# lucidrains/imagen-pytorch

Hardware: AMD Instinct MI355X
Metric: images/sec (64->256 cascade, 1000 steps, bs=8) (higher is better)
Workload: dtype f16; 1 GPU; C3: README unet1 (dim 32, 64^2) + unet2 (dim 32, 256^2, lowres_cond) cascade, 1000 DDPM steps/stage, CFG 3.0, dynamic thresholding, batch 8 per GPU; global_batch=8, parallelism=batch-sharded x1, one RCCL all-gather of final images, batch_schedule=5 whole cascades side by side (one stream each), images_in_flight=40, denoiser_evals_per_image=4000

## Files before the change

### imagen-pytorch_amd/csrc/elementwise.hip

```cpp
#include <algorithm>
#include <cstdint>
#include <cstdlib>
#include "common.h"
#include "gca_device.h"

namespace {

__device__ __forceinline__ int lanes_per_row(int groups) {
  int l = 1;
  while (l < groups && l < 64) l <<= 1;
  return l;
}

__device__ __forceinline__ float group_sum(float v, int lpr) {
  for (int off = lpr >> 1; off > 0; off >>= 1) v += __shfl_xor(v, off);
  return v;
}

__global__ __launch_bounds__(256) void rowstat_kernel(const ImagenRowstatParams p, int lpr) {
  const int rows_per_block = 256 / lpr;
  const int sub = threadIdx.x / lpr, li = threadIdx.x % lpr;
  const int r = blockIdx.x * rows_per_block + sub;
  if (r >= p.rows) return;
  const int b = r / p.rows_per_batch, rr = r - b * p.rows_per_batch;
// ... 478 lines not shown
  s_b2[t] = bias2;
  float a = 0.f;
#pragma unroll
  for (int j = 0; j < kGcaFastP; ++j) {
    const int i = sl + j * nsl;
    a += pv[j] * (i < chunks ? s_wgt[i] : 0.f);
  }
  for (int i = sl + kGcaFastP * nsl; i < chunks; i += nsl) a += part[(size_t)i * stride + 2 + c] * s_wgt[i];
  float* red_f = reinterpret_cast<float*>(s_red);
  red_f[t] = a;
  __syncthreads();
  if (t < C) {
    float v = 0.f;
    for (int q = 0; q < nsl; ++q) v += red_f[q * C + t];
    s_ctx[t] = v * inv_S;
  }
  __syncthreads();
  GCA_STAMP(5);
  gca_fast_matvec<W>(w1, w1t, C, hidden, s_ctx, s_red, [&](int o, float v) __attribute__((always_inline)) { s_hid[o] = silu_f(v + s_b1[o]); });
  GCA_STAMP(6);
  gca_fast_matvec<W>(w2, w2t, hidden, C, s_hid, s_red, [&](int o, float v) __attribute__((always_inline)) {
    const float g = sigmoid_f(v + s_b2[o]);
    gate_a[o] = g;
    if (gate_b) gate_b[o] = g;
  });
  GCA_STAMP(7);
}

__global__ __launch_bounds__(kGcaFastThreads) void gca_final_fast_kernel(const ImagenGcaFinalParams p) {
  GCA_STAMP(0);
  gca_final_fast_body<kGcaFastW>(p.part, p.w1t, p.b1, p.w2t, p.b2, blockIdx.x, p.C, p.hidden, p.chunks, p.gate + (size_t)blockIdx.x * p.C, nullptr);
}

template <int PHASE>
__global__ __launch_bounds__(256) void gca_final_split_kernel(const ImagenGcaFinalParams p) {
  __shared__ float s_in[1024], s_wgt[1024], s_red[kGcaScratchFloats];
  const int tid = threadIdx.x, b = blockIdx.y;
  if constexpr (PHASE == 1) {
    gca_merge(p.part + (size_t)b * p.chunks * (p.C + 2), p.chunks, p.C, s_in, s_wgt, s_red);
    const int o = blockIdx.x * 32 + (tid & 31), sl = tid >> 5;
    float a = 0.f;
    if (o < p.hidden) {
      const float* w = p.w1t + o;
#pragma unroll 8
      for (int c = sl; c < p.C; c += 8) a += w[(size_t)c * p.hidden] * s_in[c];
    }
    s_red[tid] = a;
    __syncthreads();
    if (tid < 32 && o < p.hidden) {
      float t = 0.f;
#pragma unroll
      for (int q = 0; q < 8; ++q) t += s_red[q * 32 + tid];
      p.hid[(size_t)b * p.hidden + o] = silu_f(t + p.b1[o]);
    }
  } else {
    for (int i = tid; i < p.hidden; i += 256) s_in[i] = p.hid[(size_t)b * p.hidden + i];
    __syncthreads();
    const int c = blockIdx.x * 64 + (tid & 63), sl = tid >> 6;
    float a = 0.f;
    if (c < p.C) {
      const float* w = p.w2t + c;
#pragma unroll 8
      for (int o = sl; o < p.hidden; o += 4) a += w[(size_t)o * p.C] * s_in[o];
    }
    s_red[tid] = a;
    __syncthreads();
    if (tid < 64 && c < p.C) p.gate[(size_t)b * p.C + c] = sigmoid_f(s_red[tid] + s_red[64 + tid] + s_red[128 + tid] + s_red[192 + tid] + p.b2[c]);
  }
}

__global__ __launch_bounds__(kGcaFastThreads) void gca_tail_kernel(const ImagenGcaTailParams p) {
  GCA_STAMP(0);
  __shared__ float s_gate[1024];
  const int t = threadIdx.x, b = blockIdx.y;
  const int C = p.C, lpr = C >> 3;
  const int rpp = kGcaFastThreads / lpr;
  const int per = (p.HW + (int)gridDim.x - 1) / (int)gridDim.x;
  const int r_begin = blockIdx.x * per, r_end = min(r_begin + per, p.HW);
  const int g = t & (lpr - 1), sub = t / lpr;
  const f16* hb = reinterpret_cast<const f16*>(p.h) + (size_t)b * p.HW * p.ld_h + g * 8;
  const f16* rb = reinterpret_cast<const f16*>(p.res) + (size_t)b * p.HW * p.ld_res + g * 8;
  f16* ob = reinterpret_cast<f16*>(p.out) + (size_t)b * p.HW * p.ld_out + g * 8;
  f16* ab = p.act_out ? reinterpret_cast<f16*>(p.act_out) + (size_t)b * p.HW * p.ld_act + g * 8 : nullptr;
  int r = r_begin + sub;
  f16x8 hv = {}, rv = {};
  if (r < r_end) {
    hv = *reinterpret_cast<const f16x8*>(hb + (size_t)r * p.ld_h);
    rv = *reinterpret_cast<const f16x8*>(rb + (size_t)r * p.ld_res);
  }
  if (p.part) {
    gca_final_fast_body<6>(p.part, p.w1t, p.b1, p.w2t, p.b2, b, C, p.hidden, p.chunks, s_gate, (p.gate && blockIdx.x == 0) ? p.gate + (size_t)b * C : nullptr);
  } else {
    if (t < C) s_gate[t] = p.gate_in ? p.gate_in[(size_t)b * C + t] : 1.0f;
    __syncthreads();
  }
  float4 pa0 = make_float4(0.f, 0.f, 0.f, 0.f), pa1 = pa0;
  if (p.act_pa) {
    pa0 = *reinterpret_cast<const float4*>(p.act_pa + g * 8);
    pa1 = *reinterpret_cast<const float4*>(p.act_pa + g * 8 + 4);
  }
  const float4 g0 = *reinterpret_cast<const float4*>(s_gate + g * 8), g1 = *reinterpret_cast<const float4*>(s_gate + g * 8 + 4);
  const float gt[8] = {g0.x, g0.y, g0.z, g0.w, g1.x, g1.y, g1.z, g1.w};
  const float pa[8] = {pa0.x, pa0.y, pa0.z, pa0.w, pa1.x, pa1.y, pa1.z, pa1.w};
  const float inv_c = 1.0f / (float)C;
  while (r < r_end) {
    const int rn = r + rpp;
    f16x8 hn = {}, rnx = {};
    if (rn < r_end) {
      hn = *reinterpret_cast<const f16x8*>(hb + (size_t)rn * p.ld_h);
      rnx = *reinterpret_cast<const f16x8*>(rb + (size_t)rn * p.ld_res);
    }
    f16x8 o;
    float vr[8], ssq = 0.f, sum = 0.f;
#pragma unroll
    for (int j = 0; j < 8; ++j) {
      o[j] = (f16)((float)hv[j] * gt[j] + (float)rv[j]);
      vr[j] = (float)o[j];
      ssq += vr[j] * vr[j];
      sum += vr[j];
    }
    *reinterpret_cast<f16x8*>(ob + (size_t)r * p.ld_out) = o;
    const size_t row = (size_t)b * p.HW + r;
    if (p.ssq_out || ab) {
      const float tot = group_sum(ssq, lpr);
      if (p.ssq_out && g == 0) p.ssq_out[row] = tot;
      if (ab) {
        const float rs = __builtin_amdgcn_rsqf(fmaxf(tot, 1e-24f));
        f16x8 a;
#pragma unroll
        for (int j = 0; j < 8; ++j) a[j] = (f16)silu_f(vr[j] * rs * pa[j]);
        *reinterpret_cast<f16x8*>(ab + (size_t)r * p.ld_act) = a;
      }
    }
    if (p.mu_out) {
      const float mean = group_sum(sum, lpr) * inv_c;
      float q = 0.f;
#pragma unroll
      for (int j = 0; j < 8; ++j) { const float d = vr[j] - mean; q += d * d; }
      const float var = group_sum(q, lpr) * inv_c;
      if (g == 0) {
        p.mu_out[row] = mean;
        p.rs_out[row] = rsqrtf(var + p.eps);
      }
    }
    hv = hn;
    rv = rnx;
    r = rn;
  }
  GCA_STAMP(8);
}

__global__ __launch_bounds__(256) void time_embed_kernel(const ImagenTimeEmbedParams p) {
  const int i = blockIdx.x * 256 + threadIdx.x;
  if (i >= p.B * p.out_dim) return;
  const int b = i / p.out_dim, o = i - b * p.out_dim;
  int st = p.step_ptr ? *p.step_ptr : 0;
  if (p.steps > 0) st = min(max(st, 0), p.steps - 1);
  const float x = p.step_ptr ? p.coef[(size_t)st * 8 + 6] : p.times[b];
  const int nf = 2 * p.half_dim + 1;
  const float* w = p.w + (size_t)o * nf;
  float a = p.bias[o] + w[0] * x;
  for (int k = 0; k < p.half_dim; ++k) {
    const float f = x * p.freqs[k] * 6.283185307179586f;
    a += w[1 + k] * sinf(f) + w[1 + p.half_dim + k] * cosf(f);
  }
  reinterpret_cast<f16*>(p.hid)[(size_t)b * p.ld_hid + o] = (f16)silu_f(a);
}

__global__ __launch_bounds__(256) void scale_shift_kernel(const ImagenScaleShiftParams p) {
  const int i = blockIdx.x * 256 + threadIdx.x;
  if (i >= p.B * p.total_c) return;
  const int b = i / p.total_c, c = i - b * p.total_c;
  float sc, sh;
  if (p.ss_f32) {
    const float* ss = reinterpret_cast<const float*>(p.ss) + (size_t)b * p.ld_ss;
    sc = ss[p.idx_scale[c]];
    sh = ss[p.idx_shift[c]];
  } else {
    const f16* ss = reinterpret_cast<const f16*>(p.ss) + (size_t)b * p.ld_ss;
    sc = (float)ss[p.idx_scale[c]];
    sh = (float)ss[p.idx_shift[c]];
  }
  p.pa[i] = p.gamma_s[c] * (sc + 1.0f);
  p.ps[i] = sh;
}

constexpr int kLfRows = 16, kLfKc = 128;

__global__ __launch_bounds__(256) void linear_f32_kernel(const ImagenLinearF32Params p) {
  __shared__ float xs[kLfRows][kLfKc];
  const int o = blockIdx.x * 256 + threadIdx.x;
  const int r0 = blockIdx.y * kLfRows;
  const int nr = min(kLfRows, p.rows - r0);
  float acc[kLfRows];
#pragma unroll
  for (int j = 0; j < kLfRows; ++j) acc[j] = 0.f;
  for (int k0 = 0; k0 < p.K; k0 += kLfKc) {
    const int kc = min(kLfKc, p.K - k0);
    __syncthreads();
    for (int i = threadIdx.x; i < kLfRows * kLfKc; i += 256) {
      const int j = i / kLfKc, k = i - j * kLfKc;
      float v = 0.f;
      if (j < nr && k < kc) {
        const size_t at = (size_t)(r0 + j) * p.ld_x + k0 + k;
        v = p.x_f32 ? reinterpret_cast<const float*>(p.x)[at] : (float)reinterpret_cast<const f16*>(p.x)[at];
        if (p.act_in == IMAGEN_ACT_SILU) v = silu_f(v);
      }
      xs[j][k] = v;
    }
    __syncthreads();
    if (o < p.Cout) {
      const float* w = p.wt + (size_t)k0 * p.Cout + o;
      for (int k = 0; k < kc; ++k) {
        const float wv = w[(size_t)k * p.Cout];
#pragma unroll
        for (int j = 0; j < kLfRows; ++j) acc[j] = fmaf(xs[j][k], wv, acc[j]);
      }
    }
  }
  if (o >= p.Cout) return;
  const float b = p.bias ? p.bias[o] : 0.f;
  for (int j = 0; j < nr; ++j) {
    float v = acc[j] + b;
    if (p.res) v += (float)reinterpret_cast<const f16*>(p.res)[(size_t)(r0 + j) * p.ld_res + o];
    p.y[(size_t)(r0 + j) * p.ld_y + o] = v;
  }
}

__global__ __launch_bounds__(256) void pack_image_kernel(const ImagenPackImageParams p) {
  const int i = blockIdx.x * 256 + threadIdx.x;
  const int HW = p.H * p.W;
  if (i >= p.B * p.Brep * HW) return;
  const int bo = i / HW, px = i - bo * HW;
  const int bs = bo % p.B;
  f16* out = reinterpret_cast<f16*>(p.out) + (size_t)i * p.Cpad;
  for (int c = 0; c < p.Cpad; ++c) {
    float v = 0.f;
    if (c < p.Ca) v = p.a[((size_t)bs * p.Ca + c) * HW + px];
    else if (c - p.Ca < p.Cb) v = p.b[((size_t)bs * p.Cb + (c - p.Ca)) * HW + px];
    out[c] = (f16)v;
  }
}

__global__ __launch_bounds__(256) void rows_copy_kernel(const ImagenRowsCopyParams p) {
  const int groups = p.C >> 3;
  const int i = blockIdx.x * 256 + threadIdx.x;
  if (i >= p.B * p.rows * groups) return;
  const int g = i % groups;
  const int r = (i / groups) % p.rows;
  const int b = i / (groups * p.rows);
  const f16* s = reinterpret_cast<const f16*>(p.src) + (size_t)b * p.src_bs + (size_t)r * p.src_rs + g * 8;
  f16* d = reinterpret_cast<f16*>(p.dst) + (size_t)b * p.dst_bs + (size_t)r * p.dst_rs + g * 8;
  *reinterpret_cast<uint4*>(d) = *reinterpret_cast<const uint4*>(s);
}

__global__ __launch_bounds__(256) void select_rows_kernel(const ImagenSelectRowsParams p) {
  const int groups = p.C >> 3;
  const int i = blockIdx.x * 256 + threadIdx.x;
  if (i >= p.R * p.L * groups) return;
  const int g = i % groups;
  const int l = (i / groups) % p.L;
  const int r = i / (groups * p.L);
  const int sb = p.src[r];
  const bool take = p.keep[r] && (p.mask == nullptr || p.mask[(size_t)sb * p.L + l]);
  const f16* s = take ? reinterpret_cast<const f16*>(p.a) + ((size_t)sb * p.L + l) * p.C + g * 8
                      : reinterpret_cast<const f16*>(p.nul) + (size_t)l * p.C + g * 8;
  *reinterpret_cast<uint4*>(reinterpret_cast<f16*>(p.dst) + ((size_t)r * p.L + l) * p.C + g * 8) = *reinterpret_cast<const uint4*>(s);
}

__global__ __launch_bounds__(256) void mean_rows_kernel(const ImagenMeanRowsParams p) {
  const int groups = p.C >> 3;
  const int i = blockIdx.x * 256 + threadIdx.x;
  if (i >= p.B * groups) return;
  const int b = i / groups, g = i - b * groups;
  const f16* x = reinterpret_cast<const f16*>(p.x) + (size_t)b * p.bs_x + g * 8;
  float acc[8] = {0, 0, 0, 0, 0, 0, 0, 0};
  for (int r = 0; r < p.rows; ++r) {
    const f16x8 v = *reinterpret_cast<const f16x8*>(x + (size_t)r * p.ld_x);
#pragma unroll
    for (int j = 0; j < 8; ++j) acc[j] += (float)v[j];
  }
  f16x8 o;
  const float inv = 1.0f / (float)p.rows;
#pragma unroll
  for (int j = 0; j < 8; ++j) o[j] = (f16)(acc[j] * inv);
  *reinterpret_cast<f16x8*>(reinterpret_cast<f16*>(p.out) + (size_t)b * p.ld_out + g * 8) = o;
}

__global__ __launch_bounds__(256) void memset32_kernel(uint32_t* dst, uint32_t value, int count) {
  const int i = blockIdx.x * 256 + threadIdx.x;
  if (i < count) dst[i] = value;
}

inline bool al8(long v) { return v % 8 == 0; }
inline bool al16(const void* q) { return (reinterpret_cast<uintptr_t>(q) & 15) == 0; }
constexpr long kIntMax = 2147483647L;

int host_lpr(int groups) {
  int l = 1;
  while (l < groups && l < 64) l <<= 1;
  return l;
}

__global__ __launch_bounds__(256) void act_prep_kernel(const ImagenActPrepParams p) {
  constexpr int U = 4;
  const int gpp = (p.C1 + p.C2) >> 3;
  const long total = (long)p.rows * gpp;
  const f16* x1 = reinterpret_cast<const f16*>(p.x1);
  const f16* x2 = reinterpret_cast<const f16*>(p.x2);
  f16* y = reinterpret_cast<f16*>(p.y);
  const long stride = (long)gridDim.x * 256;
  for (long i0 = (long)blockIdx.x * 256 + threadIdx.x; i0 < total; i0 += stride * U) {
    f16x8 in[U];
    float rs[U], mu[U], qb[U];
    float4 a0[U], a1[U], s0[U], s1[U];
    f16* dst[U];
#pragma unroll
    for (int u = 0; u < U; ++u) {
      const long i = i0 + u * stride;
      const bool ok = i < total;
      const long ii = ok ? i : 0;
      const int r = (int)(ii / gpp), g = (int)(ii - (long)r * gpp);
      const int b = r / p.rows_per_batch, rr = r - b * p.rows_per_batch;
      const int c0 = g * 8;
      const f16* src = c0 < p.C1 ? x1 + (size_t)b * p.bs1 + (size_t)rr * p.ld1 + c0 : x2 + (size_t)b * p.bs2 + (size_t)rr * p.ld2 + (c0 - p.C1);
      in[u] = *reinterpret_cast<const f16x8*>(src);
      rs[u] = p.rs ? p.rs[r] : (p.ssq_a ? p.ssq_a[r] : 1.0f);
      qb[u] = (!p.rs && p.ssq_b) ? p.ssq_b[r] : 0.0f;
      mu[u] = p.mu ? p.mu[r] : 0.0f;
      const float* pa = p.pa ? p.pa + (size_t)b * p.pstride + c0 : nullptr;
      const float* ps = p.ps ? p.ps + (size_t)b * p.pstride + c0 : nullptr;
      a0[u] = pa ? *reinterpret_cast<const float4*>(pa) : make_float4(1.f, 1.f, 1.f, 1.f);
      a1[u] = pa ? *reinterpret_cast<const float4*>(pa + 4) : make_float4(1.f, 1.f, 1.f, 1.f);
      s0[u] = ps ? *reinterpret_cast<const float4*>(ps) : make_float4(0.f, 0.f, 0.f, 0.f);
      s1[u] = ps ? *reinterpret_cast<const float4*>(ps + 4) : make_float4(0.f, 0.f, 0.f, 0.f);
      dst[u] = ok ? y + (size_t)b * p.bsy + (size_t)rr * p.ldy + c0 : nullptr;
    }
#pragma unroll
    for (int u = 0; u < U; ++u) {
      if (!dst[u]) continue;
      float sc = rs[u];
      if (!p.rs && p.ssq_a) sc = __builtin_amdgcn_rsqf(fmaxf(rs[u] + p.ssq_wb * qb[u], 1e-24f));
      const float a[8] = {a0[u].x, a0[u].y, a0[u].z, a0[u].w, a1[u].x, a1[u].y, a1[u].z, a1[u].w};
      const float sh[8] = {s0[u].x, s0[u].y, s0[u].z, s0[u].w, s1[u].x, s1[u].y, s1[u].z, s1[u].w};
      f16x8 out;
#pragma unroll
      for (int j = 0; j < 8; ++j) {
        float v = ((float)in[u][j] - mu[u]) * sc * a[j] + sh[j];
        if (p.act_in == IMAGEN_ACT_SILU) v = silu_f(v);
        else if (p.act_in == IMAGEN_ACT_GELU) v = gelu_f(v);
        out[j] = (f16)v;
      }
      *reinterpret_cast<f16x8*>(dst[u]) = out;
    }
  }
}

template <int L>
__global__ __launch_bounds__(256) void act_prep_stat_kernel(const ImagenActPrepParams p) {
  const int gpp = (p.C1 + p.C2) >> 3;
  const int g = threadIdx.x % L;
  const int r = blockIdx.x * (256 / L) + threadIdx.x / L;
  const bool live = r < p.rows && g < gpp;
  const int rc = min(r, p.rows - 1), gc = min(g, gpp - 1);
  const int b = rc / p.rows_per_batch, rr = rc - b * p.rows_per_batch;
  const int c0 = gc * 8;
  const f16* x1 = reinterpret_cast<const f16*>(p.x1);
  const f16* x2 = reinterpret_cast<const f16*>(p.x2);
  const f16* src = c0 < p.C1 ? x1 + (size_t)b * p.bs1 + (size_t)rr * p.ld1 + c0 : x2 + (size_t)b * p.bs2 + (size_t)rr * p.ld2 + (c0 - p.C1);
  const f16x8 in = *reinterpret_cast<const f16x8*>(src);
  const float qb = p.ssq_b ? p.ssq_b[rc] : 0.0f;
  const float* pa = p.pa ? p.pa + (size_t)b * p.pstride + c0 : nullptr;
  const float* ps = p.ps ? p.ps + (size_t)b * p.pstride + c0 : nullptr;
  const float4 a0 = pa ? *reinterpret_cast<const float4*>(pa) : make_float4(1.f, 1.f, 1.f, 1.f);
  const float4 a1 = pa ? *reinterpret_cast<const float4*>(pa + 4) : make_float4(1.f, 1.f, 1.f, 1.f);
  const float4 s0 = ps ? *reinterpret_cast<const float4*>(ps) : make_float4(0.f, 0.f, 0.f, 0.f);
  const float4 s1 = ps ? *reinterpret_cast<const float4*>(ps + 4) : make_float4(0.f, 0.f, 0.f, 0.f);
  float own = 0.0f;
  if (live && c0 < p.C1) {
#pragma unroll
    for (int j = 0; j < 8; ++j) own += (float)in[j] * (float)in[j];
  }
#pragma unroll
  for (int o = L / 2; o >= 1; o >>= 1) own += __shfl_xor(own, o);
  if (!live) return;
  const float sc = __builtin_amdgcn_rsqf(fmaxf(own + p.ssq_wb * qb, 1e-24f));
  const float a[8] = {a0.x, a0.y, a0.z, a0.w, a1.x, a1.y, a1.z, a1.w};
  const float sh[8] = {s0.x, s0.y, s0.z, s0.w, s1.x, s1.y, s1.z, s1.w};
  f16x8 out;
#pragma unroll
  for (int j = 0; j < 8; ++j) {
    float v = (float)in[j] * sc * a[j] + sh[j];
    if (p.act_in == IMAGEN_ACT_SILU) v = silu_f(v);
    else if (p.act_in == IMAGEN_ACT_GELU) v = gelu_f(v);
    out[j] = (f16)v;
  }
  *reinterpret_cast<f16x8*>(reinterpret_cast<f16*>(p.y) + (size_t)b * p.bsy + (size_t)rr * p.ldy + c0) = out;
}

__global__ __launch_bounds__(256) void step_slice_kernel(const ImagenStepSliceParams p) {
  int st = *p.step_ptr;
  if (p.steps > 0) st = min(max(st, 0), p.steps - 1);
  const size_t step = (size_t)st;
  const int w0 = p.words0, w1 = w0 + p.words1, w2 = w1 + p.words2, tot = w2 + p.words3;
  for (int i = blockIdx.x * 256 + threadIdx.x; i < tot; i += gridDim.x * 256) {
    const uint4* s;
    uint4* d;
    int j, w;
    if (i < w0) { s = reinterpret_cast<const uint4*>(p.src0); d = reinterpret_cast<uint4*>(p.dst0); j = i; w = p.words0; }
    else if (i < w1) { s = reinterpret_cast<const uint4*>(p.src1); d = reinterpret_cast<uint4*>(p.dst1); j = i - w0; w = p.words1; }
    else if (i < w2) { s = reinterpret_cast<const uint4*>(p.src2); d = reinterpret_cast<uint4*>(p.dst2); j = i - w1; w = p.words2; }
    else { s = reinterpret_cast<const uint4*>(p.src3); d = reinterpret_cast<uint4*>(p.dst3); j = i - w2; w = p.words3; }
    d[j] = s[step * (size_t)w + j];
  }
}

}

#ifdef GCA_TRACE
extern "C" int imagen_debug_gca_trace(void* buf) { return (int)hipMemcpyToSymbol(HIP_SYMBOL(g_gca_trace), &buf, sizeof(buf)); }
#endif

int launch_step_slice(const ImagenStepSliceParams* p, hipStream_t s) {
  IMAGEN_CHECK(p->step_ptr && p->words0 > 0 && p->src0 && p->dst0, "step_slice: null step_ptr / first segment");
  IMAGEN_CHECK((!p->words1 || (p->src1 && p->dst1)) && (!p->words2 || (p->src2 && p->dst2)) && (!p->words3 || (p->src3 && p->dst3)),
               "step_slice: a segment with words but no pointers");
  const long tot = (long)p->words0 + p->words1 + p->words2 + p->words3;
  hipLaunchKernelGGL(step_slice_kernel, dim3((unsigned)std::min<long>((tot + 255) / 256, 2048L)), dim3(256), 0, s, *p);
  return imagen_hip_status("step_slice");
}

int launch_rowstat(const ImagenRowstatParams* p, hipStream_t s) {
  IMAGEN_CHECK(p->C1 % 8 == 0 && p->C2 % 8 == 0 && p->ld1 % 8 == 0, "rowstat: channels/stride must be multiples of 8");
  IMAGEN_CHECK(p->rows > 0 && p->rows_per_batch > 0, "rowstat: empty");
  IMAGEN_CHECK(p->x1 && p->rs && p->C1 > 0 && (!p->x2 || p->C2 > 0) && p->mode >= 0 && p->mode <= 2 && (p->mode != 1 || p->mu),
               "rowstat: null x1 / rs (mode 1: mu), no channels or mode %d", p->mode);
  IMAGEN_CHECK(al8(p->bs1) && al16(p->x1) && (!p->x2 || (al8(p->ld2) && al8(p->bs2) && al16(p->x2))),
               "rowstat: strides must be multiples of 8 and the rows 16-byte aligned (bs1=%d ld2=%d bs2=%d)", p->bs1, p->ld2, p->bs2);
  const int lpr = host_lpr((p->C1 + (p->x2 ? p->C2 : 0)) / 8);
  const int rpb = 256 / lpr;
  hipLaunchKernelGGL(rowstat_kernel, dim3((p->rows + rpb - 1) / rpb), dim3(256), 0, s, *p, lpr);
  return imagen_hip_status("rowstat");
}

int launch_gate_residual(const ImagenGateResidualParams* p, hipStream_t s) {
  IMAGEN_CHECK(p->C % 8 == 0, "gate_residual: C %% 8");
  IMAGEN_CHECK(p->h && p->res && p->out && p->C > 0 && p->rows > 0 && p->rows_per_batch > 0, "gate_residual: null tensors / empty problem");
  IMAGEN_CHECK(al8(p->ld_h) && al8(p->ld_res) && al8(p->ld_out) && al16(p->h) && al16(p->res) && al16(p->out) && (!p->gate || al16(p->gate)),
               "gate_residual: row strides must be multiples of 8 and the rows 16-byte aligned (ld_h=%d ld_res=%d ld_out=%d)", p->ld_h, p->ld_res, p->ld_out);
  const int lpr = host_lpr(p->C / 8);
  const int rpb = 256 / lpr;
  hipLaunchKernelGGL(gate_residual_kernel, dim3((p->rows + rpb - 1) / rpb), dim3(256), 0, s, *p, lpr);
  return imagen_hip_status("gate_residual");
}

int launch_ln_residual(const ImagenLnResidualParams* p, hipStream_t s) {
  IMAGEN_CHECK(p->C % 8 == 0, "ln_residual: C %% 8");
  IMAGEN_CHECK(p->y && p->g && p->out && p->C > 0 && p->rows > 0 && p->rows_per_batch > 0, "ln_residual: null tensors / empty problem");
  IMAGEN_CHECK(!p->mu_out == !p->rs_out, "ln_residual: mu_out and rs_out come together");
  IMAGEN_CHECK(al8(p->ld_y) && al8(p->bs_y) && al8(p->ld_out) && al8(p->bs_out) && al16(p->y) && al16(p->out) &&
                   (!p->res || (al8(p->ld_res) && al8(p->bs_res) && al16(p->res))),
               "ln_residual: strides must be multiples of 8 and the rows 16-byte aligned (ld_y=%d bs_y=%d ld_res=%d bs_res=%d ld_out=%d bs_out=%d)", p->ld_y,
               p->bs_y, p->ld_res, p->bs_res, p->ld_out, p->bs_out);
  const int lpr = host_lpr(p->C / 8);
  const int rpb = 256 / lpr;
  hipLaunchKernelGGL(ln_residual_kernel, dim3((p->rows + rpb - 1) / rpb), dim3(256), 0, s, *p, lpr);
  return imagen_hip_status("ln_residual");
}

int launch_qnorm(const ImagenQnormParams* p, hipStream_t s) {
  IMAGEN_CHECK(p->q && p->q_scale && p->rows > 0 && p->heads > 0, "qnorm: null tensors / empty problem");
  IMAGEN_CHECK(p->head_dim == 0 || p->head_dim == 32 || p->head_dim == 64, "qnorm: head_dim %d", p->head_dim);
  IMAGEN_CHECK(al8(p->ld) && al16(p->q) && p->ld >= p->heads * (p->head_dim == 32 ? 32 : 64), "qnorm: row stride %d must be a multiple of 8 covering the %d heads, rows 16-byte aligned",
               p->ld, p->heads);
  IMAGEN_CHECK((long)p->rows * p->heads <= kIntMax - 64, "qnorm: rows * heads does not fit an int");
  const int items = p->rows * p->heads;
  hipLaunchKernelGGL(qnorm_kernel, dim3((items + 31) / 32), dim3(256), 0, s, *p);
  return imagen_hip_status("qnorm");
}

static int check_kv_prep(const ImagenKvPrepParams* p) {
  IMAGEN_CHECK(p->rows > 0 && p->B > 0 && p->heads > 0 && p->r0 >= 0, "kv_prep: empty");
  IMAGEN_CHECK(p->k_src && p->v_src && p->k_scale && p->khat && p->vt, "kv_prep: null pointer");
  IMAGEN_CHECK(p->head_dim == 0 || p->head_dim == 32 || p->head_dim == 64, "kv_prep: head_dim %d", p->head_dim);
  IMAGEN_CHECK(al8(p->k_bs) && al8(p->k_hs) && al8(p->k_rs) && al16(p->khat), "kv_prep: K-hat strides must be multiples of 8, rows 16-byte aligned (%d %d %d)",
               p->k_bs, p->k_hs, p->k_rs);
  IMAGEN_CHECK(p->src_is_f32 || (al8(p->src_bs) && al8(p->src_rs) && al8(p->src_hs) && al16(p->k_src) && al16(p->v_src)),
               "kv_prep: fp16 source strides / offsets must be multiples of 8 (%d %d %d)", p->src_bs, p->src_rs, p->src_hs);
  IMAGEN_CHECK((long)p->B * p->heads <= 65535, "kv_prep: B * heads = %ld exceeds the grid", (long)p->B * p->heads);
  return 0;
}

int launch_kv_prep(const ImagenKvPrepParams* p, hipStream_t s) {
  if (check_kv_prep(p) != 0) return -1;
  hipLaunchKernelGGL(kv_prep_kernel, dim3((p->rows + 31) / 32, p->B * p->heads), dim3(256), 0, s, *p);
  return imagen_hip_status("kv_prep");
}

int launch_kv_prep_multi(const ImagenKvPrepMultiParams* p, hipStream_t s) {
  IMAGEN_CHECK(p->jobs && p->n > 0 && p->max_rows > 0 && p->max_bh > 0, "kv_prep_multi: empty");
  hipLaunchKernelGGL(kv_prep_multi_kernel, dim3((p->max_rows + 31) / 32, p->max_bh, p->n), dim3(256), 0, s, *p);
  return imagen_hip_status("kv_prep_multi");
}

int launch_gca_partial(const ImagenGcaPartialParams* p, hipStream_t s) {
  IMAGEN_CHECK(p->C % 8 == 0 && p->C / 8 <= 256, "gca: unsupported C %d", p->C);
  const int chunk_px = (p->HW + p->chunks - 1) / p->chunks;
  const int groups = p->C / 8;
  if (p->w1t) {
    IMAGEN_CHECK((groups & (groups - 1)) == 0 && groups <= 64, "gca: in-kernel finalisation needs a power-of-two C/8 (C = %d)", p->C);
    IMAGEN_CHECK(p->b1 && p->w2t && p->b2 && p->gate && p->hidden > 0, "gca: incomplete finalisation parameters");
    IMAGEN_CHECK(p->chunks == 1, "gca: in-kernel finalisation needs one chunk per image (got %d)", p->chunks);
    IMAGEN_CHECK(p->C + p->hidden + p->chunks + kGcaScratchFloats <= 2048, "gca: finalisation scratch too large (C %d hidden %d chunks %d)", p->C,
                 p->hidden, p->chunks);
  }
  if ((groups & (groups - 1)) == 0 && groups <= 64) {
    hipLaunchKernelGGL(gca_partial_online_kernel, dim3(p->chunks, p->B), dim3(256), 0, s, *p, chunk_px);
    return imagen_hip_status("gca_partial");
  }
  IMAGEN_CHECK(chunk_px <= kGcaMaxChunk, "gca: chunk of %d pixels too large", chunk_px);
  hipLaunchKernelGGL(gca_partial_kernel, dim3(p->chunks, p->B), dim3(256), 0, s, *p, chunk_px);
  return imagen_hip_status("gca_partial");
}

int launch_gca_final(const ImagenGcaFinalParams* p, hipStream_t s) {
  auto pow2 = [](int v) { return v > 0 && (v & (v - 1)) == 0; };
  IMAGEN_CHECK(p->phase >= 0 && p->phase <= 2, "gca_final: phase %d", p->phase);
  if (p->phase != 0) {
    IMAGEN_CHECK(p->hid && p->C <= 1024 && p->hidden <= 1024 && p->chunks <= 1024 && p->C % 2 == 0, "gca_final: the two-phase finalisation needs hid, C / hidden / chunks <= 1024 (got %d / %d / %d)", p->C, p->hidden, p->chunks);
    if (p->phase == 1) hipLaunchKernelGGL(gca_final_split_kernel<1>, dim3((p->hidden + 31) / 32, p->B), dim3(256), 0, s, *p);
    else hipLaunchKernelGGL(gca_final_split_kernel<2>, dim3((p->C + 63) / 64, p->B), dim3(256), 0, s, *p);
    return imagen_hip_status("gca_final");
  }
  if (pow2(p->C) && pow2(p->hidden) && p->C >= 4 && p->C <= 1024 && p->hidden >= 4 && p->hidden <= 1024 && p->chunks <= 1024) {
    hipLaunchKernelGGL(gca_final_fast_kernel, dim3(p->B), dim3(kGcaFastThreads), 0, s, *p);
    return imagen_hip_status("gca_final");
  }
  const size_t sm = (size_t)(p->C + p->hidden + p->chunks + kGcaScratchFloats) * sizeof(float);
  hipLaunchKernelGGL(gca_final_kernel, dim3(p->B), dim3(256), sm, s, *p);
  return imagen_hip_status("gca_final");
}

int launch_gca_tail(const ImagenGcaTailParams* p, hipStream_t s) {
  auto pow2 = [](int v) { return v > 0 && (v & (v - 1)) == 0; };
  IMAGEN_CHECK(p->h && p->res && p->out && p->B > 0 && p->HW > 0, "gca_tail: null tensors / empty problem");
  IMAGEN_CHECK(pow2(p->C) && p->C >= 8 && p->C <= 512, "gca_tail: C %d must be a power of two in [8, 512]", p->C);
  IMAGEN_CHECK(!p->part || (p->w1t && p->b1 && p->w2t && p->b2 && pow2(p->hidden) && p->hidden >= 4 && p->hidden <= 1024 && p->chunks >= 1 && p->chunks <= 1024),
               "gca_tail: GlobalContext finalisation needs the squeeze MLP, a power-of-two hidden width (%d) and 1..1024 chunks (%d)", p->hidden, p->chunks);
  IMAGEN_CHECK(p->ld_h % 8 == 0 && p->ld_res % 8 == 0 && p->ld_out % 8 == 0 && (!p->act_out || (p->act_pa && p->ld_act % 8 == 0)),
               "gca_tail: row strides must be multiples of 8 (act_out needs act_pa)");
  IMAGEN_CHECK(!p->mu_out == !p->rs_out, "gca_tail: mu_out and rs_out come together");
  IMAGEN_CHECK(p->slabs >= 1 && p->slabs <= 65535, "gca_tail: slabs %d", p->slabs);
  hipLaunchKernelGGL(gca_tail_kernel, dim3(p->slabs, p->B), dim3(kGcaFastThreads), 0, s, *p);
  return imagen_hip_status("gca_tail");
}

int launch_time_embed(const ImagenTimeEmbedParams* p, hipStream_t s) {
  IMAGEN_CHECK(p->freqs && p->w && p->bias && p->hid && (p->step_ptr ? p->coef != nullptr : p->times != nullptr), "time_embed: null pointer");
  IMAGEN_CHECK(p->B > 0 && p->out_dim > 0 && p->half_dim >= 0 && p->ld_hid >= p->out_dim && (long)p->B * p->out_dim <= kIntMax - 256, "time_embed: bad shape");
  const int n = p->B * p->out_dim;
  hipLaunchKernelGGL(time_embed_kernel, dim3((n + 255) / 256), dim3(256), 0, s, *p);
  return imagen_hip_status("time_embed");
}

int launch_scale_shift(const ImagenScaleShiftParams* p, hipStream_t s) {
  IMAGEN_CHECK(p->ss && p->gamma_s && p->idx_scale && p->idx_shift && p->pa && p->ps, "scale_shift: null pointer");
  IMAGEN_CHECK(p->B > 0 && p->total_c > 0 && (long)p->B * p->total_c <= kIntMax - 256, "scale_shift: bad shape");
  const int n = p->B * p->total_c;
  hipLaunchKernelGGL(scale_shift_kernel, dim3((n + 255) / 256), dim3(256), 0, s, *p);
  return imagen_hip_status("scale_shift");
}

int launch_linear_f32(const ImagenLinearF32Params* p, hipStream_t s) {
  IMAGEN_CHECK(p->x && p->wt && p->y, "linear_f32: null pointer");
  IMAGEN_CHECK(p->rows > 0 && p->K > 0 && p->Cout > 0 && p->ld_x >= p->K && p->ld_y >= p->Cout && (!p->res || p->ld_res >= p->Cout), "linear_f32: bad shape");
  IMAGEN_CHECK(p->act_in == IMAGEN_ACT_NONE || p->act_in == IMAGEN_ACT_SILU, "linear_f32: input activation none | SiLU");
  IMAGEN_CHECK((p->rows + kLfRows - 1) / kLfRows <= 65535, "linear_f32: %d rows", p->rows);
  hipLaunchKernelGGL(linear_f32_kernel, dim3((p->Cout + 255) / 256, (p->rows + kLfRows - 1) / kLfRows), dim3(256), 0, s, *p);
  return imagen_hip_status("linear_f32");
}

int launch_pack_image(const ImagenPackImageParams* p, hipStream_t s) {
  IMAGEN_CHECK(p->a && p->out && (p->Cb == 0 || p->b), "pack_image: null pointer");
  IMAGEN_CHECK(p->B > 0 && p->Brep > 0 && p->H > 0 && p->W > 0 && p->Ca > 0 && p->Cb >= 0 && p->Cpad > 0 && p->Ca + p->Cb <= p->Cpad,
               "pack_image: bad shape (Ca=%d Cb=%d Cpad=%d)", p->Ca, p->Cb, p->Cpad);
  IMAGEN_CHECK((long)p->B * p->Brep * p->H * p->W <= kIntMax - 256, "pack_image: B * Brep * H * W does not fit an int");
  const int n = p->B * p->Brep * p->H * p->W;
  hipLaunchKernelGGL(pack_image_kernel, dim3((n + 255) / 256), dim3(256), 0, s, *p);
  return imagen_hip_status("pack_image");
}

int launch_rows_copy(const ImagenRowsCopyParams* p, hipStream_t s) {
  IMAGEN_CHECK(p->C % 8 == 0, "rows_copy: C %% 8");
  IMAGEN_CHECK(p->src && p->dst && p->B > 0 && p->rows > 0 && p->C > 0, "rows_copy: null tensors / empty problem");
  IMAGEN_CHECK(al8(p->src_bs) && al8(p->src_rs) && al8(p->dst_bs) && al8(p->dst_rs) && al16(p->src) && al16(p->dst),
               "rows_copy: strides and offsets must be multiples of 8 (src %d %d, dst %d %d)", p->src_bs, p->src_rs, p->dst_bs, p->dst_rs);
  IMAGEN_CHECK((long)p->B * p->rows * (p->C / 8) <= kIntMax - 256, "rows_copy: B * rows * C / 8 does not fit an int");
  const int n = p->B * p->rows * (p->C / 8);
  hipLaunchKernelGGL(rows_copy_kernel, dim3((n + 255) / 256), dim3(256), 0, s, *p);
  return imagen_hip_status("rows_copy");
}

int launch_select_rows(const ImagenSelectRowsParams* p, hipStream_t s) {
  IMAGEN_CHECK(p->C % 8 == 0, "select_rows: C %% 8");
  IMAGEN_CHECK(p->a && p->nul && p->src && p->keep && p->dst && p->R > 0 && p->L > 0 && p->C > 0, "select_rows: null tensors / empty problem");
  IMAGEN_CHECK(al16(p->a) && al16(p->nul) && al16(p->dst), "select_rows: rows must be 16-byte aligned");
  IMAGEN_CHECK((long)p->R * p->L * (p->C / 8) <= kIntMax - 256, "select_rows: R * L * C / 8 does not fit an int");
  const int n = p->R * p->L * (p->C / 8);
  hipLaunchKernelGGL(select_rows_kernel, dim3((n + 255) / 256), dim3(256), 0, s, *p);
  return imagen_hip_status("select_rows");
}

int launch_mean_rows(const ImagenMeanRowsParams* p, hipStream_t s) {
  IMAGEN_CHECK(p->C % 8 == 0 && p->rows > 0, "mean_rows: bad shape");
  IMAGEN_CHECK(p->x && p->out && p->B > 0 && p->C > 0, "mean_rows: null tensors / empty problem");
  IMAGEN_CHECK(al8(p->bs_x) && al8(p->ld_x) && al8(p->ld_out) && al16(p->x) && al16(p->out), "mean_rows: strides must be multiples of 8 (bs_x=%d ld_x=%d ld_out=%d)",
               p->bs_x, p->ld_x, p->ld_out);
  IMAGEN_CHECK((long)p->B * (p->C / 8) <= kIntMax - 256, "mean_rows: B * C / 8 does not fit an int");
  const int n = p->B * (p->C / 8);
  hipLaunchKernelGGL(mean_rows_kernel, dim3((n + 255) / 256), dim3(256), 0, s, *p);
  return imagen_hip_status("mean_rows");
}

int launch_memset32(const ImagenMemset32Params* p, hipStream_t s) {
  IMAGEN_CHECK(p->dst && p->count > 0 && p->count <= kIntMax - 255, "memset32: null dst or a count (%d) outside [1, 2^31 - 256]", p->count);
  hipLaunchKernelGGL(memset32_kernel, dim3((p->count + 255) / 256), dim3(256), 0, s, reinterpret_cast<uint32_t*>(p->dst), p->value,
                     p->count);
  return imagen_hip_status("memset32");
}

int launch_act_prep(const ImagenActPrepParams* p, hipStream_t s) {
  IMAGEN_CHECK(p->x1 && p->y && p->rows > 0 && p->rows_per_batch > 0, "act_prep: null x1/y or empty problem");
  IMAGEN_CHECK(p->C1 % 8 == 0 && p->C2 % 8 == 0 && p->ld1 % 8 == 0 && p->ldy % 8 == 0 && (!p->x2 || p->ld2 % 8 == 0) && (p->x2 || p->C2 == 0),
               "act_prep: channel counts / strides must be multiples of 8 (C1=%d C2=%d ld1=%d ld2=%d ldy=%d)", p->C1, p->C2, p->ld1, p->ld2, p->ldy);
  const long total = (long)p->rows * ((p->C1 + p->C2) >> 3);
  const int blocks = (int)std::min<long>((total + 1023) / 1024, 256L * 8);
  if (p->self_stat) {
    IMAGEN_CHECK(!p->rs && !p->mu && !p->ssq_a, "act_prep: self_stat excludes rs / mu / ssq_a");
    const int gpp = (p->C1 + p->C2) / 8;
    IMAGEN_CHECK(gpp <= 64, "act_prep: self_stat handles at most 512 channels per pixel (got %d)", 8 * gpp);
    if (gpp <= 16) hipLaunchKernelGGL(act_prep_stat_kernel<16>, dim3((p->rows + 15) / 16), dim3(256), 0, s, *p);
    else if (gpp <= 32) hipLaunchKernelGGL(act_prep_stat_kernel<32>, dim3((p->rows + 7) / 8), dim3(256), 0, s, *p);
    else hipLaunchKernelGGL(act_prep_stat_kernel<64>, dim3((p->rows + 3) / 4), dim3(256), 0, s, *p);
    return imagen_hip_status("act_prep (self_stat)");
  }
  hipLaunchKernelGGL(act_prep_kernel, dim3(blocks), dim3(256), 0, s, *p);
  return imagen_hip_status("act_prep");
}
```

Baseline: 1.400 images/s.

## Restructure act_prep into row tiles with hoisted channel affine and templated activation

The act_prep kernel now gives each thread a fixed channel group and walks whole rows in contiguous tiles per workgroup. This replaces the flat grid-stride loop that did per-element div/mod and reloaded the per-image affine scale/shift on every element. The affine is loaded once and refreshed only when the image index changes, the activation is a template parameter, and the grid is capped at CUs times a workgroups-per-CU factor. The risks are idle lanes when 256 is not a multiple of the channel groups, and the per-image affine reload inside the loop on image boundaries.

```diff
diff --git a/imagen-pytorch_amd/csrc/elementwise.hip b/imagen-pytorch_amd/csrc/elementwise.hip
--- a/imagen-pytorch_amd/csrc/elementwise.hip
+++ b/imagen-pytorch_amd/csrc/elementwise.hip
@@ -804,56 +804,105 @@
   return l;
 }
 
-__global__ __launch_bounds__(256) void act_prep_kernel(const ImagenActPrepParams p) {
-  constexpr int U = 4;
+constexpr int kPrepU = 4;
+#ifndef ACT_PREP_WG_PER_CU
+#define ACT_PREP_WG_PER_CU 8
+#endif
+
+struct PrepWalk {
+  int r, b, rr;
+};
+__device__ __forceinline__ PrepWalk prep_walk_start(int r, int rows_per_batch) {
+  PrepWalk w;
+  w.r = r;
+  w.b = r / rows_per_batch;
+  w.rr = r - w.b * rows_per_batch;
+  return w;
+}
+__device__ __forceinline__ void prep_walk_advance(PrepWalk& w, int step, int rows_per_batch) {
+  w.r += step;
+  w.rr += step;
+  while (w.rr >= rows_per_batch) {
+    w.rr -= rows_per_batch;
+    ++w.b;
+  }
+}
+
+__device__ __forceinline__ void prep_affine(const ImagenActPrepParams& p, int b, int c0, float (&a)[8], float (&sh)[8]) {
+  const float* pa = p.pa ? p.pa + (size_t)b * p.pstride + c0 : nullptr;
+  const float* ps = p.ps ? p.ps + (size_t)b * p.pstride + c0 : nullptr;
+  const float4 a0 = pa ? *reinterpret_cast<const float4*>(pa) : make_float4(1.f, 1.f, 1.f, 1.f);
+  const float4 a1 = pa ? *reinterpret_cast<const float4*>(pa + 4) : make_float4(1.f, 1.f, 1.f, 1.f);
+  const float4 s0 = ps ? *reinterpret_cast<const float4*>(ps) : make_float4(0.f, 0.f, 0.f, 0.f);
+  const float4 s1 = ps ? *reinterpret_cast<const float4*>(ps + 4) : make_float4(0.f, 0.f, 0.f, 0.f);
+  a[0] = a0.x; a[1] = a0.y; a[2] = a0.z; a[3] = a0.w; a[4] = a1.x; a[5] = a1.y; a[6] = a1.z; a[7] = a1.w;
+  sh[0] = s0.x; sh[1] = s0.y; sh[2] = s0.z; sh[3] = s0.w; sh[4] = s1.x; sh[5] = s1.y; sh[6] = s1.z; sh[7] = s1.w;
+}
+
+template <int ACT>
+__device__ __forceinline__ f16x8 prep_apply(const f16x8& in, float mu, float sc, const float (&a)[8], const float (&sh)[8]) {
+  f16x8 out;
+#pragma unroll
+  for (int j = 0; j < 8; ++j) {
+    float v = ((float)in[j] - mu) * sc * a[j] + sh[j];
+    if (ACT == IMAGEN_ACT_SILU) v = silu_f(v);
+    else if (ACT == IMAGEN_ACT_GELU) v = gelu_f(v);
+    out[j] = (f16)v;
+  }
+  return out;
+}
+
+__device__ __forceinline__ void prep_tile_range(int ntiles, int& t0, int& t1) {
+  t0 = (int)((long)blockIdx.x * ntiles / gridDim.x);
+  t1 = (int)((long)(blockIdx.x + 1) * ntiles / gridDim.x);
+}
+
+template <int ACT>
+__global__ __launch_bounds__(256) void act_prep_kernel(const ImagenActPrepParams p, int ntiles) {
+  constexpr int U = kPrepU;
   const int gpp = (p.C1 + p.C2) >> 3;
-  const long total = (long)p.rows * gpp;
-  const f16* x1 = reinterpret_cast<const f16*>(p.x1);
-  const f16* x2 = reinterpret_cast<const f16*>(p.x2);
-  f16* y = reinterpret_cast<f16*>(p.y);
-  const long stride = (long)gridDim.x * 256;
-  for (long i0 = (long)blockIdx.x * 256 + threadIdx.x; i0 < total; i0 += stride * U) {
+  const int rpt = 256 / gpp;
+  const int rl = (int)threadIdx.x / gpp, g = (int)threadIdx.x - rl * gpp;
+  const bool active = rl < rpt;
+  const int c0 = g * 8;
+  const bool from1 = c0 < p.C1;
+  const f16* xg = from1 ? reinterpret_cast<const f16*>(p.x1) + c0 : reinterpret_cast<const f16*>(p.x2) + (c0 - p.C1);
+  const int ld = from1 ? p.ld1 : p.ld2, bs = from1 ? p.bs1 : p.bs2;
+  f16* yg = reinterpret_cast<f16*>(p.y) + c0;
+  const bool per_image = p.pstride != 0 && (p.pa || p.ps);
+  float a[8], sh[8];
+  int ab = 0;
+  prep_affine(p, 0, c0, a, sh);
+  int t0, t1;
+  prep_tile_range(ntiles, t0, t1);
+  PrepWalk w = prep_walk_start(t0 * rpt + rl, p.rows_per_batch);
+  for (int t = t0; t < t1; t += U) {
     f16x8 in[U];
     float rs[U], mu[U], qb[U];
-    float4 a0[U], a1[U], s0[U], s1[U];
+    int ib[U];
     f16* dst[U];
 #pragma unroll
     for (int u = 0; u < U; ++u) {
-      const long i = i0 + u * stride;
-      const bool ok = i < total;
-      const long ii = ok ? i : 0;
-      const int r = (int)(ii / gpp), g = (int)(ii - (long)r * gpp);
-      const int b = r / p.rows_per_batch, rr = r - b * p.rows_per_batch;
-      const int c0 = g * 8;
-      const f16* src = c0 < p.C1 ? x1 + (size_t)b * p.bs1 + (size_t)rr * p.ld1 + c0 : x2 + (size_t)b * p.bs2 + (size_t)rr * p.ld2 + (c0 - p.C1);
-      in[u] = *reinterpret_cast<const f16x8*>(src);
+      const bool ok = active && t + u < t1 && w.r < p.rows;
+      const int r = ok ? w.r : 0, b = ok ? w.b : 0, rr = ok ? w.rr : 0;
+      in[u] = *reinterpret_cast<const f16x8*>(xg + (size_t)b * bs + (size_t)rr * ld);
       rs[u] = p.rs ? p.rs[r] : (p.ssq_a ? p.ssq_a[r] : 1.0f);
       qb[u] = (!p.rs && p.ssq_b) ? p.ssq_b[r] : 0.0f;
       mu[u] = p.mu ? p.mu[r] : 0.0f;
-      const float* pa = p.pa ? p.pa + (size_t)b * p.pstride + c0 : nullptr;
-      const float* ps = p.ps ? p.ps + (size_t)b * p.pstride + c0 : nullptr;
-      a0[u] = pa ? *reinterpret_cast<const float4*>(pa) : make_float4(1.f, 1.f, 1.f, 1.f);
-      a1[u] = pa ? *reinterpret_cast<const float4*>(pa + 4) : make_float4(1.f, 1.f, 1.f, 1.f);
-      s0[u] = ps ? *reinterpret_cast<const float4*>(ps) : make_float4(0.f, 0.f, 0.f, 0.f);
-      s1[u] = ps ? *reinterpret_cast<const float4*>(ps + 4) : make_float4(0.f, 0.f, 0.f, 0.f);
-      dst[u] = ok ? y + (size_t)b * p.bsy + (size_t)rr * p.ldy + c0 : nullptr;
+      ib[u] = b;
+      dst[u] = ok ? yg + (size_t)b * p.bsy + (size_t)rr * p.ldy : nullptr;
+      prep_walk_advance(w, rpt, p.rows_per_batch);
     }
 #pragma unroll
     for (int u = 0; u < U; ++u) {
       if (!dst[u]) continue;
+      if (per_image && ib[u] != ab) {
+        ab = ib[u];
+        prep_affine(p, ab, c0, a, sh);
+      }
       float sc = rs[u];
       if (!p.rs && p.ssq_a) sc = __builtin_amdgcn_rsqf(fmaxf(rs[u] + p.ssq_wb * qb[u], 1e-24f));
-      const float a[8] = {a0[u].x, a0[u].y, a0[u].z, a0[u].w, a1[u].x, a1[u].y, a1[u].z, a1[u].w};
-      const float sh[8] = {s0[u].x, s0[u].y, s0[u].z, s0[u].w, s1[u].x, s1[u].y, s1[u].z, s1[u].w};
-      f16x8 out;
-#pragma unroll
-      for (int j = 0; j < 8; ++j) {
-        float v = ((float)in[u][j] - mu[u]) * sc * a[j] + sh[j];
-        if (p.act_in == IMAGEN_ACT_SILU) v = silu_f(v);
-        else if (p.act_in == IMAGEN_ACT_GELU) v = gelu_f(v);
-        out[j] = (f16)v;
-      }
-      *reinterpret_cast<f16x8*>(dst[u]) = out;
+      *reinterpret_cast<f16x8*>(dst[u]) = prep_apply<ACT>(in[u], mu[u], sc, a, sh);
     }
   }
 }
@@ -900,6 +949,28 @@
   *reinterpret_cast<f16x8*>(reinterpret_cast<f16*>(p.y) + (size_t)b * p.bsy + (size_t)rr * p.ldy + c0) = out;
 }
 
+int prep_num_cus() {
+  static int cached[16] = {};
+  int dev = 0, v = 0;
+  (void)hipGetDevice(&dev);
+  const bool slot = dev >= 0 && dev < 16;
+  if (slot && cached[dev]) return cached[dev];
+  if (hipDeviceGetAttribute(&v, hipDeviceAttributeMultiprocessorCount, dev) != hipSuccess || v < 1) v = 256;
+  if (slot) cached[dev] = v;
+  return v;
+}
+
+int act_prep_grid(const ImagenActPrepParams& p, int* tile_rows, int* ntiles) {
+  const int gpp = (p.C1 + p.C2) / 8;
+  const int rpt = p.self_stat ? 256 / (gpp <= 16 ? 16 : gpp <= 32 ? 32 : 64) : 256 / gpp;
+  const int nt = (p.rows + rpt - 1) / rpt;
+  if (tile_rows) *tile_rows = rpt;
+  if (ntiles) *ntiles = nt;
+  if (p.self_stat) return nt;
+  const int cap = prep_num_cus() * ACT_PREP_WG_PER_CU;
+  return std::min((nt + kPrepU - 1) / kPrepU, cap);
+}
+
 __global__ __launch_bounds__(256) void step_slice_kernel(const ImagenStepSliceParams p) {
   int st = *p.step_ptr;
   if (p.steps > 0) st = min(max(st, 0), p.steps - 1);
@@ -1135,17 +1206,30 @@
   IMAGEN_CHECK(p->x1 && p->y && p->rows > 0 && p->rows_per_batch > 0, "act_prep: null x1/y or empty problem");
   IMAGEN_CHECK(p->C1 % 8 == 0 && p->C2 % 8 == 0 && p->ld1 % 8 == 0 && p->ldy % 8 == 0 && (!p->x2 || p->ld2 % 8 == 0) && (p->x2 || p->C2 == 0),
                "act_prep: channel counts / strides must be multiples of 8 (C1=%d C2=%d ld1=%d ld2=%d ldy=%d)", p->C1, p->C2, p->ld1, p->ld2, p->ldy);
-  const long total = (long)p->rows * ((p->C1 + p->C2) >> 3);
-  const int blocks = (int)std::min<long>((total + 1023) / 1024, 256L * 8);
+  const int gpp = (p->C1 + p->C2) / 8;
+  IMAGEN_CHECK(gpp >= 1 && gpp <= 256 && p->rows <= kIntMax - 4096 && p->act_in >= IMAGEN_ACT_NONE && p->act_in <= IMAGEN_ACT_GELU,
+               "act_prep: 8 .. 2048 channels per pixel, at most 2^31 - 4097 rows, act_in none / SiLU / GELU (got %d channels, %d rows, act_in %d)",
+               8 * gpp, p->rows, p->act_in);
   if (p->self_stat) {
     IMAGEN_CHECK(!p->rs && !p->mu && !p->ssq_a, "act_prep: self_stat excludes rs / mu / ssq_a");
-    const int gpp = (p->C1 + p->C2) / 8;
     IMAGEN_CHECK(gpp <= 64, "act_prep: self_stat handles at most 512 channels per pixel (got %d)", 8 * gpp);
-    if (gpp <= 16) hipLaunchKernelGGL(act_prep_stat_kernel<16>, dim3((p->rows + 15) / 16), dim3(256), 0, s, *p);
-    else if (gpp <= 32) hipLaunchKernelGGL(act_prep_stat_kernel<32>, dim3((p->rows + 7) / 8), dim3(256), 0, s, *p);
-    else hipLaunchKernelGGL(act_prep_stat_kernel<64>, dim3((p->rows + 3) / 4), dim3(256), 0, s, *p);
+  }
+  int ntiles = 0;
+  const int grid = act_prep_grid(*p, nullptr, &ntiles);
+  if (p->self_stat) {
+    if (gpp <= 16) hipLaunchKernelGGL(act_prep_stat_kernel<16>, dim3(grid), dim3(256), 0, s, *p);
+    else if (gpp <= 32) hipLaunchKernelGGL(act_prep_stat_kernel<32>, dim3(grid), dim3(256), 0, s, *p);
+    else hipLaunchKernelGGL(act_prep_stat_kernel<64>, dim3(grid), dim3(256), 0, s, *p);
     return imagen_hip_status("act_prep (self_stat)");
   }
-  hipLaunchKernelGGL(act_prep_kernel, dim3(blocks), dim3(256), 0, s, *p);
+  if (p->act_in == IMAGEN_ACT_SILU) hipLaunchKernelGGL(act_prep_kernel<IMAGEN_ACT_SILU>, dim3(grid), dim3(256), 0, s, *p, ntiles);
+  else if (p->act_in == IMAGEN_ACT_GELU) hipLaunchKernelGGL(act_prep_kernel<IMAGEN_ACT_GELU>, dim3(grid), dim3(256), 0, s, *p, ntiles);
+  else hipLaunchKernelGGL(act_prep_kernel<IMAGEN_ACT_NONE>, dim3(grid), dim3(256), 0, s, *p, ntiles);
   return imagen_hip_status("act_prep");
 }
+
+extern "C" int imagen_debug_act_prep_grid(const ImagenActPrepParams* p, int* tile_rows, int* ntiles) {
+  const int gpp = (p->C1 + p->C2) / 8;
+  if (gpp < 1 || gpp > 256 || p->rows < 1 || (p->self_stat && gpp > 64)) return -1;
+  return act_prep_grid(*p, tile_rows, ntiles);
+}
```

New measurement: 1.406 images/s (median of 6 runs). No clear change (+0.4%).
